# lh3/minigraph

Measured on NVIDIA H100. Metric: mapped Gbp/s (-cx lr), higher is better.
Workload: dtype int64/u8 (fp32 chain penalties, bit-exact)

## Files before the change

### minigraph_b200/csrc/mgb_engine.cu

```cuda
#include <stdio.h>
#include <stdlib.h>
#include <string.h>
#include <math.h>
#include <vector>
#include <array>
#include <memory>
#include <algorithm>
#include <string>
#include <chrono>
#include <thread>
#include <mutex>
#include <condition_variable>
#include <functional>
#include <unordered_map>
#include "mgb_hostpool.h"

#include "../../include/mgb200.h"
#include "mgb_galign.cuh"
#include "mgb_gaf.cuh"
#include "mgb_ingest.cuh"

#ifndef MGB_HOSTSIM
#include <cuda_runtime.h>
#include "mgb_index.cuh"
// ... 2377 lines not shown
		const TestTier &t;
		int32_t *smem;
		MG_HD void put(int i, int64_t rc, int64_t s, int64_t n_iter, int64_t n_cigar, int lane) const
		{
			if (lane == 0) { int64_t *o = t.out + 4 * (int64_t)i; o[0] = rc, o[1] = s, o[2] = n_iter, o[3] = n_cigar; }
		}
		MG_HD int run(int i, Arena &A, WfTbJob *tb, int lane) const
		{
			WfResult r;
			const char *ts_i = t.ts + t.t_off[i], *qs_i = t.qs + t.q_off[i];
			int64_t cont_cells = 0;
			const int rc = t.tier == 1? wfa_smem<WfTier1::W_, WfTier1::MAXLEN_, WfTier1::TBCAP_>(A, smem, t.tl[i], ts_i, t.ql[i], qs_i, &r, lane)
					: t.tier == 2? wfa_smem<WfTier2::W_, WfTier2::MAXLEN_, WfTier2::TBCAP_>(A, smem, t.tl[i], ts_i, t.ql[i], qs_i, &r, lane)
								 : wfa_smem<WfTier2::W_, WfTier2::MAXLEN_, WfTier2::TBCAP_, true>(A, smem, t.tl[i], ts_i, t.ql[i], qs_i, &r, lane, &cont_cells);
			if (rc == 1) put(i, 1, -1, 0, 0, lane);
			if (rc != 0) return rc < 0? rc : 0;
			wfa_tb_keep(tb, r, t.tl[i], ts_i, t.ql[i], qs_i, i, lane);
			return 1;
		}
		MG_HD int done(const WfTbJob &b, int lane) const
		{
			if (b.rc < 0) return b.rc;
			if (b.n_cigar > t.cap) return MGB_E_INTERNAL;
			for (int32_t j = lane; j < b.n_cigar; j += MGB_W) t.cigar[b.job * t.cap + j] = b.cig[b.first + j];
			put((int)b.job, 0, b.s, b.n_iter, b.n_cigar, lane);
			return 0;
		}
		MG_HD void fail(int i, int rc, int lane) const { put(i, rc, -1, 0, 0, lane); }
		MG_HD void traced(unsigned long long, int) const {}
	};
	MG_HD int operator()(int w, int32_t *smem, Arena &A, int, int lane) const
	{
		const Gaps g{*this, smem};
		WfaBatch<Gaps> batch;
		batch.open(A);
		for (int i = w; i < n; i += n_workers) batch.add(g, i, A, lane);
		batch.flush(g, A, lane);
		warp_sync();
		return 0;
	}
};

static int test_wfa_tier_impl(int tier, int n, const char *ts, const int64_t *t_off, const int32_t *tl, const char *qs, const int64_t *q_off,
							  const int32_t *ql, int64_t *out, uint32_t *cigar, int cap)
{
	if ((tier != 1 && tier != 2 && tier != MGB_TEST_TIER2_CONT) || n < 0 || cap < 0) {
		set_error("mgb_test_wfa_tier: tier must be 1, 2 or MGB_TEST_TIER2_CONT, n and cap at least 0");
		return MGB_E_UNSUPPORTED;
	}
	for (int i = 0; i < n; ++i)
		if (tl[i] < 1 || ql[i] < 1 || t_off[i] < 0 || q_off[i] < 0) { set_error("mgb_test_wfa_tier: gap " + std::to_string(i) + " has an empty side"); return MGB_E_UNSUPPORTED; }
	if (n == 0) return 0;
	if (int e = test_no_device()) return e;
	auto ts_d = upload(ts, test_seq_bytes(n, t_off, tl)), qs_d = upload(qs, test_seq_bytes(n, q_off, ql));
	auto t_off_d = upload(t_off, n), q_off_d = upload(q_off, n);
	auto tl_d = upload(tl, n), ql_d = upload(ql, n);
	DevBuf<int64_t> out_d(4 * (size_t)n);
	DevBuf<uint32_t> cigar_d((size_t)n * cap + 1);
	TestTier t;
	const int warps = tier == 1? StageSpec<S_WFA_SMALL>::warps : StageSpec<S_WFA_MID>::warps;
	t.tier = tier, t.cap = cap, t.n = n, t.n_workers = (std::min(n, 64 * warps) + warps - 1) / warps * warps;
	t.ts = ts_d, t.qs = qs_d, t.t_off = t_off_d, t.q_off = q_off_d, t.tl = tl_d, t.ql = ql_d, t.out = out_d, t.cigar = cigar_d;
	const uint64_t arena_bytes = tier == MGB_TEST_TIER2_CONT? (uint64_t)5 << 20 : (uint64_t)256 << 10;
	const int rc = tier == 1? test_launch<S_WFA_SMALL>(t.n_workers, t.n_workers, arena_bytes, t)
							: test_launch<S_WFA_MID>(t.n_workers, t.n_workers, arena_bytes, t);
	if (rc) return rc;
	d2h(out, out_d, sizeof(int64_t) * 4 * (size_t)n);
	d2h(cigar, cigar_d, sizeof(uint32_t) * (size_t)n * cap);
	return 0;
}

extern "C" int mgb_test_wfa_tier(int tier, int n, const char *ts, const int64_t *t_off, const int32_t *tl, const char *qs, const int64_t *q_off,
								 const int32_t *ql, int64_t *out, uint32_t *cigar, int cap)
{
	try { return test_wfa_tier_impl(tier, n, ts, t_off, tl, qs, q_off, ql, out, cigar, cap); } catch (const MgbError &e) { return e.code; }
}

struct TestGwfa {
	GraphDev g;
	int mode, walk_cap;
	const char *q;
	const int64_t *q_off;
	const int32_t *ql, *off0, *off1, *max_ed;
	const uint32_t *v0, *v1;
	int64_t *out;
	int32_t *walk;
	MG_HD int operator()(int i, int32_t *smem, Arena &A, int, int lane) const
	{
		GwfShared *sh = (GwfShared*)smem;
		GwfOpt opt;
		opt.traceback = 1, opt.max_chk = 1000, opt.bw_dyn = 1000, opt.max_lag = max_ed[i] / 2, opt.s_term = -1;
		opt.i_term = 500000000LL;
		A.top = 0, A.peak = 0;
		const char *q_i = q + q_off[i];
		int rc = 0;
		GwfResult rs;
		const GwfResult *r = &rs;
		if (mode == 0) {
			if (lane == 0) sh->A = A;
			warp_sync();
			rc = gwf_align_w(sh, g, opt, ql[i], q_i, v0[i], off0[i], v1[i], off1[i], max_ed[i], lane);
			r = &sh->r;
		} else {
			if (lane == 0) rc = gwf_align(A, g, opt, ql[i], q_i, v0[i], off0[i], v1[i], off1[i], max_ed[i], &rs);
			rc = warp_bcast_i32(rc, 0);
		}
		if (lane == 0) {
			int64_t *o = out + 6 * (int64_t)i;
			const int32_t nv = rc == 0 && r->s >= 0? r->nv : 0;
			if (nv > walk_cap) rc = MGB_E_INTERNAL;
			o[0] = rc;
			o[1] = rc == 0? r->s : -1, o[2] = rc == 0? (int64_t)r->end_v : -1, o[3] = rc == 0? r->end_off : -1;
			o[4] = rc == 0? nv : 0, o[5] = rc == 0? r->n_iter : 0;
			if (rc == 0) for (int32_t j = 0; j < nv; ++j) walk[(int64_t)i * walk_cap + j] = r->v[j];
		}
		warp_sync();
		return 0;
	}
};

static int test_gwfa_impl(const mg_idx_t *gi, int mode, int n, const char *q, const int64_t *q_off, const int32_t *ql, const uint32_t *v0,
						  const int32_t *off0, const uint32_t *v1, const int32_t *off1, const int32_t *max_ed, int64_t *out, int32_t *walk, int walk_cap)
{
	if (gi == 0 || (mode != 0 && mode != 1) || n < 0 || walk_cap < 0) { set_error("mgb_test_gwfa: an index, mode 0 or 1, n and walk_cap at least 0"); return MGB_E_UNSUPPORTED; }
	const Model *M = model_of(gi);
	for (int i = 0; i < n; ++i)
		if (ql[i] < 1 || q_off[i] < 0 || (v0[i] >> 1) >= (uint32_t)M->g.n_seg || (v1[i] >> 1) >= (uint32_t)M->g.n_seg || off0[i] < 0 || off0[i] >= M->seg_len[v0[i] >> 1]
			|| off1[i] < 0 || off1[i] >= M->seg_len[v1[i] >> 1]) {
			set_error("mgb_test_gwfa: bridge " + std::to_string(i) + " has an empty query or an end outside the graph");
			return MGB_E_UNSUPPORTED;
		}
	if (n == 0) return 0;
	if (int e = test_no_device(M->device)) return e;
	auto q_d = upload(q, test_seq_bytes(n, q_off, ql));
	auto q_off_d = upload(q_off, n);
	auto ql_d = upload(ql, n), off0_d = upload(off0, n), off1_d = upload(off1, n), max_ed_d = upload(max_ed, n);
	auto v0_d = upload(v0, n), v1_d = upload(v1, n);
	DevBuf<int64_t> out_d(6 * (size_t)n);
	DevBuf<int32_t> walk_d((size_t)n * walk_cap + 1);
	TestGwfa t;
	t.g = M->g, t.mode = mode, t.walk_cap = walk_cap;
	t.q = q_d, t.q_off = q_off_d, t.ql = ql_d, t.off0 = off0_d, t.off1 = off1_d, t.max_ed = max_ed_d, t.v0 = v0_d, t.v1 = v1_d, t.out = out_d, t.walk = walk_d;
	if (int e = test_launch<S_GWFA>(n, std::min(n, 8 * StageSpec<S_GWFA>::warps), (uint64_t)64 << 20, t)) return e;
	d2h(out, out_d, sizeof(int64_t) * 6 * (size_t)n);
	d2h(walk, walk_d, sizeof(int32_t) * (size_t)n * walk_cap);
	return 0;
}

extern "C" int mgb_test_gwfa(const mg_idx_t *gi, int mode, int n, const char *q, const int64_t *q_off, const int32_t *ql, const uint32_t *v0,
							 const int32_t *off0, const uint32_t *v1, const int32_t *off1, const int32_t *max_ed, int64_t *out, int32_t *walk, int walk_cap)
{
	try { return test_gwfa_impl(gi, mode, n, q, q_off, ql, v0, off0, v1, off1, max_ed, out, walk, walk_cap); } catch (const MgbError &e) { return e.code; }
}

struct TestRadix {
	u128 *a; int64_t n; int walk, hot_bytes; int32_t *rc;
	MG_HD int operator()(int, int32_t *hot, Arena &A, int, int lane) const
	{
		Arena H;
		arena_init(H, hot, hot_bytes > 0? (uint64_t)hot_bytes : 0);
		const int r = radix_sort_128x_w(hot_bytes > 0? H : A, a, n, lane, &A, walk != 0);
		if (lane == 0) *rc = r;
		return r;
	}
};

static int test_radix128_impl(u128 *a, int64_t n, int walk, int hot_bytes)
{
	if (n < 0 || hot_bytes < 0 || hot_bytes > 200 * 1024) { set_error("mgb_test_radix128: n >= 0 and 0 <= hot_bytes <= 200 KB"); return MGB_E_UNSUPPORTED; }
	if (int e = test_no_device()) return e;
	auto a_d = upload(a, n);
	DevBuf<int32_t> rc_d(1);
	TestRadix t;
	t.a = a_d, t.n = n, t.walk = walk, t.hot_bytes = hot_bytes, t.rc = rc_d;
	if (int e = test_launch<NO_STAGE>(1, 1, (uint64_t)n * 64 + (1 << 20), t, 1, hot_bytes)) return e;
	int32_t rc = 0;
	d2h(&rc, rc_d, sizeof(rc));
	if (rc == 0) d2h(a, a_d, sizeof(u128) * (size_t)n);
	return rc;
}

extern "C" int mgb_test_radix128(mg128_t *a, int64_t n, int walk, int hot_bytes)
{
	static_assert(sizeof(mg128_t) == sizeof(u128), "mg128_t and u128 are the same record");
	try { return test_radix128_impl((u128*)a, n, walk, hot_bytes); } catch (const MgbError &e) { return e.code; }
}

struct TestLchain {
	int mode;
	uint64_t slice;
	u128 *a;
	const int64_t *off;
	const int32_t *cnt;
	const LChainOpt *opt;
	int32_t *out;
	uint64_t *u;
	MG_HD int operator()(int i, int32_t *smem, Arena &A, int worker, int lane) const
	{
		A.top = 0;
		u128 *a_i = a + off[i];
		const int64_t n = cnt[i];
		const LChainOpt &co = opt[i];
		int32_t n_u = 0, n_v = 0;
		uint64_t *u_i = 0;
		int path = -1, staged = 0;
		const int rc = chain_staged(smem, slice, A, a_i, n, lane, &staged, [&](Arena &H, u128 *aw, int32_t *n_keep) {
			const int r = mode == 2? chain_run<1>(H, A, 1, co, n, aw, &n_u, &u_i, &n_v, lane, &path) : chain_run<0>(H, A, mode == 1, co, n, aw, &n_u, &u_i, &n_v, lane, &path);
			*n_keep = n_u > 0? n_v : 0;
			return r;
		});
		if (rc == 0) for (int32_t j = lane; j < n_u; j += MGB_W) u[off[i] + j] = u_i[j];
		if (lane == 0) {
			int32_t *o = out + 6 * (int64_t)i;
			o[0] = rc, o[1] = n_u, o[2] = n_v, o[3] = staged, o[4] = path, o[5] = worker;
		}
		warp_sync();
		return 0;
	}
};

static int test_lchain_impl(int mode, int n, const u128 *a, const int64_t *off, const int32_t *cnt, const mgb_lchain_opt_t *opt, int32_t *out, uint64_t *u, u128 *a_out)
{
#define MGB_SAME_FIELD(f) static_assert(offsetof(mgb_lchain_opt_t, f) == offsetof(LChainOpt, f) && sizeof(mgb_lchain_opt_t::f) == sizeof(LChainOpt::f), "mgb_lchain_opt_t and LChainOpt differ in " #f)
	MGB_SAME_FIELD(max_dist_x); MGB_SAME_FIELD(max_dist_y); MGB_SAME_FIELD(bw); MGB_SAME_FIELD(max_skip); MGB_SAME_FIELD(max_iter); MGB_SAME_FIELD(min_cnt);
	MGB_SAME_FIELD(min_sc); MGB_SAME_FIELD(pen_gap); MGB_SAME_FIELD(pen_skip); MGB_SAME_FIELD(is_cdna); MGB_SAME_FIELD(n_seg); MGB_SAME_FIELD(max_dist_inner);
	MGB_SAME_FIELD(cap_rmq_size);
#undef MGB_SAME_FIELD
	static_assert(sizeof(mgb_lchain_opt_t) == sizeof(LChainOpt), "mgb_lchain_opt_t and LChainOpt are the same record");
	if (mode < 0 || mode > 2 || n < 0) { set_error("mgb_test_lchain: mode 0, 1 or 2 and n at least 0"); return MGB_E_UNSUPPORTED; }
	int64_t max_cnt = 0;
	for (int i = 0; i < n; ++i) {
		if (cnt[i] < 0 || off[i] < 0) { set_error("mgb_test_lchain: set " + std::to_string(i) + " has a negative offset or count"); return MGB_E_UNSUPPORTED; }
		max_cnt = std::max(max_cnt, (int64_t)cnt[i]);
	}
	if (n == 0) return 0;
	if (int e = test_no_device()) return e;
	const int64_t n_a = test_seq_bytes(n, off, cnt);
	auto a_d = upload(a, n_a);
	auto off_d = upload(off, n);
	auto cnt_d = upload(cnt, n);
	auto opt_d = upload((const LChainOpt*)opt, n);
	DevBuf<int32_t> out_d(6 * (size_t)n);
	DevBuf<uint64_t> u_d((size_t)n_a + 1);
	TestLchain t;
	t.mode = mode, t.slice = mode == 2? StageSpec<S_CHAIN_RESCUE>::smem : StageSpec<S_CHAIN>::smem;
	t.a = a_d, t.off = off_d, t.cnt = cnt_d, t.opt = opt_d, t.out = out_d, t.u = u_d;
	const uint64_t arena_bytes = (uint64_t)max_cnt * 512 + ((uint64_t)1 << 20);
	const int rc = mode == 2? test_launch<S_CHAIN_RESCUE>(n, std::min(n, 2 * StageSpec<S_CHAIN_RESCUE>::warps), arena_bytes, t)
							: test_launch<S_CHAIN>(n, std::min(n, 2 * StageSpec<S_CHAIN>::warps), arena_bytes, t);
	if (rc) return rc;
	d2h(out, out_d, sizeof(int32_t) * 6 * (size_t)n);
	d2h(u, u_d, sizeof(uint64_t) * (size_t)n_a);
	d2h(a_out, a_d, sizeof(u128) * (size_t)n_a);
	return 0;
}

extern "C" int mgb_test_lchain(int mode, int n, const mg128_t *a, const int64_t *off, const int32_t *cnt, const mgb_lchain_opt_t *opt, int32_t *out,
							   uint64_t *u, mg128_t *a_out)
{
	try { return test_lchain_impl(mode, n, (const u128*)a, off, cnt, opt, out, u, (u128*)a_out); } catch (const MgbError &e) { return e.code; }
}

struct TestSketch {
	int k, w, mode;
	const char *seq;
	const int64_t *off, *pk_off, *mz_off;
	const int32_t *len;
	const uint64_t *pk;
	int32_t *out;
	u128 *mz;
	MG_HD int operator()(int i, int32_t *smem, Arena &A, int, int lane) const
	{
		A.top = 0;
		AVec<u128> mv;
		avec_init(mv);
		const char *s = seq + off[i];
		int rc = 0, path = -1;
		if (mode == 0) rc = sketch_seq_w(A, s, len[i], w, k, (uint32_t)i, mv, lane, (u128*)smem, pk_off[i] >= 0? pk + pk_off[i] : 0, &path);
		else if (lane == 0) rc = sketch_seq(A, s, len[i], w, k, (uint32_t)i, mv);
		rc = warp_bcast_i32(rc, 0);
		const int64_t n = rc == 0? (int64_t)warp_bcast_u64((uint64_t)mv.n, 0) : 0;
		if (n <= mz_off[i + 1] - mz_off[i]) {
			if (mode == 0) for (int64_t j = lane; j < n; j += MGB_W) mz[mz_off[i] + j] = mv.a[j];
			else if (lane == 0) for (int64_t j = 0; j < n; ++j) mz[mz_off[i] + j] = mv.a[j];
		}
		if (lane == 0) out[3 * (int64_t)i] = rc, out[3 * (int64_t)i + 1] = (int32_t)n, out[3 * (int64_t)i + 2] = path;
		warp_sync();
		return 0;
	}
};

static int test_sketch_impl(int k, int w, int n, const char *seq, const int64_t *off, const int32_t *len, int mode, int32_t *out, u128 *mz, const int64_t *mz_off)
{
	static_assert(SKETCH_PATH_SMEM_PK == MGB_SKETCH_PATH_SMEM_PK && SKETCH_PATH_SMEM == MGB_SKETCH_PATH_SMEM && SKETCH_PATH_ARENA == MGB_SKETCH_PATH_ARENA
				  && SKETCH_PATH_SEQ == MGB_SKETCH_PATH_SEQ, "the sketch paths of mgb200.h are mgb_seed.cuh's");
	if (k < 1 || k > 28 || w < 1 || w > 255 || (mode != 0 && mode != 1) || n < 0) {
		set_error("mgb_test_sketch: 1 <= k <= 28, 1 <= w <= 255, mode 0 or 1 and n at least 0");
		return MGB_E_UNSUPPORTED;
	}
	int32_t max_len = 0;
	for (int i = 0; i < n; ++i) {
		if (len[i] < 1 || off[i] < 0 || mz_off[i] < 0 || mz_off[i + 1] < mz_off[i]) {
			set_error("mgb_test_sketch: sequence " + std::to_string(i) + " is empty or has a bad offset");
			return MGB_E_UNSUPPORTED;
		}
		max_len = std::max(max_len, len[i]);
// ... 360 lines not shown
```

### minigraph_b200/csrc/mgb_gwfa.cuh

```cuda
#pragma once
#include "mgb_model.cuh"

namespace mgb {

static const int32_t GWF_DIAG_SHIFT = 0x40000000;

struct GwfDiag {
	uint64_t vd;
	int32_t k, len;
	uint32_t xo;
	int32_t t;
};
struct GwfIntv { uint64_t vd0, vd1; };
struct GwfTrace { int32_t v, pre; };

struct KeyDiagVd { MG_HD uint64_t operator()(const GwfDiag &p) const { return p.vd; } };
struct KeyIntvVd0 { MG_HD uint64_t operator()(const GwfIntv &p) const { return p.vd0; } };

MG_HD inline uint64_t gwf_gen_vd(uint32_t v, int32_t d) { return (uint64_t)v << 32 | (uint64_t)(uint32_t)(GWF_DIAG_SHIFT + d); }

struct U64Tab {
	uint64_t *key;
	int32_t *val, *ep;
	int32_t bits, epoch;
	int64_t n;
};

MG_HD inline uint32_t u64tab_hash(uint64_t key)
{
	key = ~key + (key << 21);
	key = key ^ key >> 24;
	key = (key + (key << 3)) + (key << 8);
	key = key ^ key >> 14;
	key = (key + (key << 2)) + (key << 4);
	key = key ^ key >> 28;
	key = key + (key << 31);
	return (uint32_t)key;
}

MG_HD MG_NOINLINE inline int u64tab_alloc(Arena &A, U64Tab &t, int bits)
{
	MGB_ALLOC(A, t.key, uint64_t, 1LL << bits);
	MGB_ALLOC(A, t.val, int32_t, 1LL << bits);
	MGB_ALLOC(A, t.ep, int32_t, 1LL << bits);
	MGB_NO_UNROLL
	for (int64_t i = 0; i < (1LL << bits); ++i) t.ep[i] = 0;
	t.bits = bits;
	return 0;
}
MG_HD inline int u64tab_init(Arena &A, U64Tab &t, int bits) { t.epoch = 1, t.n = 0; return u64tab_alloc(A, t, bits); }
MG_HD inline void u64tab_clear(U64Tab &t) { ++t.epoch, t.n = 0; }

MG_HD MG_NOINLINE inline int u64tab_grow(Arena &A, U64Tab &t)
{
	U64Tab o = t;
	MGB_TRY(u64tab_alloc(A, t, o.bits + 1));
	t.epoch = 1;
	uint64_t nmask = (1ULL << t.bits) - 1;
	MGB_NO_UNROLL
	for (int64_t i = 0; i < (1LL << o.bits); ++i) {
		if (o.ep[i] != o.epoch) continue;
		uint64_t g = u64tab_hash(o.key[i]) & nmask;
		while (t.ep[g] == t.epoch) g = (g + 1) & nmask;
		t.key[g] = o.key[i], t.val[g] = o.val[i], t.ep[g] = t.epoch;
	}
	return 0;
}

MG_HD inline int u64tab_put(Arena &A, U64Tab &t, uint64_t key, int *absent, int64_t *slot)
{
	for (;;) {
		uint64_t mask = (1ULL << t.bits) - 1, h = u64tab_hash(key) & mask;
		while (t.ep[h] == t.epoch && t.key[h] != key) h = (h + 1) & mask;
		if (t.ep[h] == t.epoch) { *absent = 0, *slot = (int64_t)h; return 0; }
		if ((uint64_t)(t.n + 1) * 2 > (1ULL << t.bits)) {
			MGB_TRY(u64tab_grow(A, t));
			continue;
		}
		t.key[h] = key, t.val[h] = 0, t.ep[h] = t.epoch, ++t.n;
		*absent = 1, *slot = (int64_t)h;
		return 0;
	}
}

struct GwfOpt { int32_t traceback, bw_dyn, max_lag, max_chk, s_term; int64_t i_term; };

struct GwfResult {
	int32_t s;
	uint32_t end_v;
	int32_t end_off, wlen, nv;
	int64_t n_iter;
	int32_t *v;
};

struct GwfState {
	const GraphDev *g;
	int32_t ql;
	const char *q;
	AVec<GwfDiag> a, B, ooo, Q;
	int64_t q_head;
	AVec<GwfIntv> intv, tmp, swap;
	AVec<GwfTrace> t;
	U64Tab ha, ht;
	int32_t s, end_tb;
};

MG_HD inline int gwf_trace_push(Arena &A, GwfState &z, int32_t v, int32_t pre, int32_t *idx)
{
	uint64_t key = (uint64_t)(uint32_t)v << 32 | (uint32_t)pre;
	int absent; int64_t slot;
	MGB_TRY(u64tab_put(A, z.ht, key, &absent, &slot));
	if (absent) {
		GwfTrace x; x.v = v, x.pre = pre;
		MGB_TRY(avec_push_c(A, z.t, x));
		z.ht.val[slot] = (int32_t)z.t.n - 1;
	}
	*idx = z.ht.val[slot];
	return 0;
}

MG_HD inline int gwf_diag_push(Arena &A, AVec<GwfDiag> &B, uint32_t v, int32_t d, int32_t k, uint32_t x, uint32_t ooo, int32_t t)
{
	GwfDiag p;
	p.vd = gwf_gen_vd(v, d), p.k = k, p.len = 0, p.xo = x << 1 | ooo, p.t = t;
	return avec_push_c(A, B, p);
}

MG_HD inline int32_t gwf_diag_update(GwfDiag *p, uint32_t v, int32_t d, int32_t k, uint32_t x, uint32_t ooo, int32_t t)
{
	uint64_t vd = gwf_gen_vd(v, d);
	if (p->vd == vd) {
		p->xo = p->k > k? p->xo : x << 1 | ooo;
		p->t = p->k > k? p->t : t;
		p->k = p->k > k? p->k : k;
		return 0;
	}
	return 1;
}

MG_HD inline int32_t gwf_extend1(int32_t d, int32_t k, int32_t vl, const char *ts, int32_t ql, const char *qs)
{
	int32_t max_k = (ql - d < vl? ql - d : vl) - 1;
	const char *ts_ = ts + 1, *qs_ = qs + d + 1;
	while (k + 4 <= max_k) {
		uint32_t x = ld32_unaligned(ts_ + k) ^ ld32_unaligned(qs_ + k);
		if (x) return k + (ctz32(x) >> 3);
		k += 4;
	}
	while (k < max_k && ts_[k] == qs_[k]) ++k;
	return k;
}

MG_HD MG_NOINLINE inline int gwf_sort_diag_cold(Arena &A, GwfDiag *c, int64_t n) { return radix_sort_exact(A, c, n, 8, KeyDiagVd()); }
MG_HD MG_NOINLINE inline int gwf_sort_intv_cold(Arena &A, GwfIntv *a, int64_t n) { return radix_sort_exact(A, a, n, 8, KeyIntvVd0()); }
// ... 181 lines not shown
		} else if (p->k == vl) {
			GwfIntv iv;
			iv.vd0 = gwf_gen_vd(v, d), iv.vd1 = iv.vd0 + 1;
			MGB_TRY(avec_push_c(A, z.tmp, iv));
		}
	}
	z.B.n += m;
	return 0;
}

MG_HD inline int gwf_ed_extend(Arena &A, GwfState &z, const GwfOpt &opt, uint32_t v1, int32_t off1, GwfResult *r)
{
	const GraphDev &g = *z.g;
	const int32_t ql = z.ql;
	const char *q = z.q;
	int32_t i, x, n = (int32_t)z.a.n, do_dedup = 1;
	r->end_v = (uint32_t)-1;
	r->end_off = z.end_tb = -1;
	z.tmp.n = 0;
	u64tab_clear(z.ha);
	z.Q.n = 0, z.q_head = 0;
	z.B.n = 0;
	MGB_TRY(avec_reserve_c(A, z.B, (int64_t)n * 2));
	GwfDiag *a = z.a.a;
	for (x = 0, i = 1; i <= n; ++i) {
		if (i == n || a[i].vd != a[i-1].vd + 1) {
			MGB_TRY(gwf_extend_batch(A, z, i - x, &a[x]));
			x = i;
		}
	}
	if (z.Q.n == 0) do_dedup = 0;

	while (z.q_head < z.Q.n) {
		GwfDiag t = z.Q.a[z.q_head++];
		uint32_t v, x0;
		int32_t ooo, d, k, vl;
		ooo = t.xo & 1, v = (uint32_t)(t.vd >> 32);
		d = (int32_t)t.vd - GWF_DIAG_SHIFT;
		k = t.k;
		vl = g_vlen(g, v);
		k = gwf_extend1(d, k, vl, g_vseq(g, v), ql, q);
		i = k + d;
		x0 = (t.xo >> 1) + ((uint32_t)(k - t.k) << 1);

		if (k + 1 < vl && i + 1 < ql) {
			int32_t push1 = 1, push2 = 1;
			if (z.B.n >= 2) push1 = gwf_diag_update(&z.B.a[z.B.n - 2], v, d-1, k+1, x0 + 1, ooo, t.t);
			if (z.B.n >= 1) push2 = gwf_diag_update(&z.B.a[z.B.n - 1], v, d,   k+1, x0 + 2, ooo, t.t);
			if (push1)          MGB_TRY(gwf_diag_push(A, z.B, v, d-1, k+1, x0 + 1, 1, t.t));
			if (push2 || push1) MGB_TRY(gwf_diag_push(A, z.B, v, d,   k+1, x0 + 2, 1, t.t));
			MGB_TRY(gwf_diag_push(A, z.B, v, d+1, k, x0 + 1, ooo, t.t));
		} else if (i + 1 < ql) {
			int32_t nv = g_arc_n(g, v), j, n_ext = 0, tw = -1;
			const DevArc *av = g_arc_a(g, v);
			GwfIntv iv;
			iv.vd0 = gwf_gen_vd(v, d), iv.vd1 = iv.vd0 + 1;
			MGB_TRY(avec_push_c(A, z.tmp, iv));
			if (opt.traceback) MGB_TRY(gwf_trace_push(A, z, (int32_t)v, t.t, &tw));
			for (j = 0; j < nv; ++j) {
				uint32_t w = av[j].w;
				int32_t ol = av[j].ow;
				int absent; int64_t slot;
				MGB_TRY(u64tab_put(A, z.ha, (uint64_t)w << 32 | (uint64_t)(uint32_t)(i + 1), &absent, &slot));
				if (q[i + 1] == g_vseq(g, w)[ol]) {
					++n_ext;
					if (absent) {
						GwfDiag p;
						p.vd = gwf_gen_vd(w, i + 1 - ol), p.k = ol, p.xo = (x0 + 2) << 1 | 1, p.t = tw, p.len = 0;
						MGB_TRY(avec_push_c(A, z.Q, p));
					}
				} else if (absent) {
					MGB_TRY(gwf_diag_push(A, z.B, w, i - ol,     ol, x0 + 1, 1, tw));
					MGB_TRY(gwf_diag_push(A, z.B, w, i + 1 - ol, ol, x0 + 2, 1, tw));
				}
			}
			if (nv == 0 || n_ext != nv)
				MGB_TRY(gwf_diag_push(A, z.B, v, d+1, k, x0 + 1, 1, t.t));
		} else if (v1 == (uint32_t)-1 || (v == v1 && k == off1)) {
			r->end_v = v, r->end_off = k, r->wlen = (int32_t)(x0 - (uint32_t)i - 1), z.end_tb = t.t;
			z.a.n = 0;
			return 0;
		} else if (k + 1 < vl) {
			MGB_TRY(gwf_diag_push(A, z.B, v, d-1, k+1, x0 + 1, ooo, t.t));
		} else if (v != v1) {
			int32_t nv = g_arc_n(g, v), j, tw = -1;
			const DevArc *av = g_arc_a(g, v);
			if (opt.traceback) MGB_TRY(gwf_trace_push(A, z, (int32_t)v, t.t, &tw));
			for (j = 0; j < nv; ++j)
				MGB_TRY(gwf_diag_push(A, z.B, av[j].w, i - av[j].ow, av[j].ow, x0 + 1, 1, tw));
		}
	}
	n = (int32_t)z.B.n;
	if (do_dedup) MGB_TRY(gwf_dedup(A, z, n, z.B.a, &n));
	if (opt.max_lag > 0 && n > opt.max_chk && ((z.s + 1) & 0xf) == 0)
		n = gwf_prune(n, z.B.a, (uint32_t)opt.max_lag, opt.bw_dyn);
	z.B.n = n;
	{ AVec<GwfDiag> sw = z.a; z.a = z.B; z.B = sw; }
	return 0;
}

MG_HD inline int gwf_align(Arena &A, const GraphDev &g, const GwfOpt &opt, int32_t ql, const char *q, uint32_t v0, int32_t off0,
						   uint32_t v1, int32_t off1, int32_t s_term, GwfResult *r)
{
	uint64_t mark = A.top;
	GwfState z;
	z.g = &g, z.ql = ql, z.q = q, z.s = 0, z.end_tb = -1, z.q_head = 0;
	avec_init(z.a), avec_init(z.B), avec_init(z.ooo), avec_init(z.Q), avec_init(z.intv), avec_init(z.tmp), avec_init(z.swap), avec_init(z.t);
	uint64_t mark_keep = mark;
	MGB_TRY(u64tab_init(A, z.ha, 6));
	MGB_TRY(u64tab_init(A, z.ht, 6));
	MGB_TRY(avec_reserve_c(A, z.t, 16));
	{
		GwfDiag d0;
		d0.vd = gwf_gen_vd(v0, -off0), d0.k = off0 - 1, d0.xo = 0, d0.len = 0, d0.t = 0;
		if (opt.traceback) MGB_TRY(gwf_trace_push(A, z, -1, -1, &d0.t));
		MGB_TRY(avec_push_c(A, z.a, d0));
	}
	if (s_term < 0 && opt.s_term >= 0) s_term = opt.s_term;
	r->n_iter = 0, r->nv = 0, r->v = 0, r->end_v = (uint32_t)-1, r->end_off = -1, r->wlen = 0;
	while (z.a.n > 0) {
		MGB_TRY(gwf_ed_extend(A, z, opt, v1, off1, r));
		r->n_iter += z.a.n;
		if (r->end_off >= 0 || z.a.n == 0) break;
		if (s_term >= 0 && z.s >= s_term) break;
		if (opt.i_term > 0 && r->n_iter > opt.i_term) break;
		++z.s;
	}
	if (opt.traceback && r->end_off >= 0) {
		int32_t i = z.end_tb, n = 1;
		while (i >= 0 && z.t.a[i].v >= 0) ++n, i = z.t.a[i].pre;
		int32_t *tmpw, *walk = (int32_t*)(A.base + mark);
		MGB_ALLOC(A, tmpw, int32_t, n);
		i = z.end_tb, n = 0;
		tmpw[n++] = (int32_t)r->end_v;
		while (i >= 0 && z.t.a[i].v >= 0) tmpw[n++] = z.t.a[i].v, i = z.t.a[i].pre;
		r->nv = n;
		for (i = 0; i < n >> 1; ++i) { int32_t x = tmpw[i]; tmpw[i] = tmpw[n - 1 - i], tmpw[n - 1 - i] = x; }
		for (i = 0; i < n; ++i) { int32_t x = tmpw[i]; walk[i] = x; }
		r->v = walk;
		mark_keep = mark + (((uint64_t)n * 4 + 15) & ~(uint64_t)15);
	}
	r->s = r->end_v != (uint32_t)-1? z.s : -1;
	A.top = mark_keep;
	return 0;
}


struct GwfShared {
	Arena A;
	GwfState z;
	GwfResult r;
};

MG_HD inline int gwf_extend_batch_w(GwfShared *sh, int32_t n, GwfDiag *a, int lane)
{
	GwfState &z = sh->z;
	const GraphDev &g = *z.g;
	const uint32_t v = (uint32_t)(a->vd >> 32);
	const int32_t vl = g_vlen(g, v), ql = z.ql;
	const char *ts = g_vseq(g, v);
	MGB_NO_UNROLL
	for (int32_t j = lane; j < n; j += MGB_W) {
		GwfDiag p = a[j];
		int32_t k = gwf_extend1((int32_t)p.vd - GWF_DIAG_SHIFT, p.k, vl, ts, ql, z.q);
		p.len = k - p.k;
		p.xo += (uint32_t)p.len << 2;
		p.k = k;
		a[j] = p;
	}
	int rc = 0;
	if (lane == 0) {
		rc = avec_reserve_c(sh->A, z.B, z.B.n + n + 2);
		if (rc == 0) rc = avec_reserve_c(sh->A, z.Q, z.Q.n + n);
		if (rc == 0) rc = avec_reserve_c(sh->A, z.tmp, z.tmp.n + n + 2);
	}
	warp_sync();
	rc = warp_bcast_i32(rc, 0);
	if (rc < 0) return rc;
	GwfDiag *b = &z.B.a[z.B.n];
	GwfDiag *Q = z.Q.a;
	GwfIntv *T = z.tmp.a;
	int64_t qn = z.Q.n, tn = z.tmp.n;
	int32_t m = 0;
	MGB_NO_UNROLL
	for (int32_t base = 0; base < n + 2; base += MGB_W) {
		const int32_t j = base + lane;
		GwfDiag p;
		int keep = 0, ends = 0;
		p.vd = 0, p.k = 0, p.xo = 0, p.t = 0, p.len = 0;
		if (j < n + 2) {
			if (j == 0) {
				p.vd = a[0].vd - 1, p.xo = a[0].xo + 2, p.k = a[0].k + 1, p.t = a[0].t;
			} else if (j == n + 1) {
				p.vd = a[n-1].vd + 1, p.xo = a[n-1].xo + 2, p.k = a[n-1].k, p.t = a[n-1].t;
			} else if (j == 1) {
				const int first = n == 1 || a[0].k > a[1].k;
				p.vd = a[0].vd;
				p.xo = first? a[0].xo + 4 : a[1].xo + 2;
				p.t = first? a[0].t : a[1].t;
				p.k = (first? a[0].k : a[1].k) + 1;
			} else if (j == n) {
				const int first = a[n-2].k > a[n-1].k + 1;
				p.vd = a[n-1].vd;
				p.xo = first? a[n-2].xo + 2 : a[n-1].xo + 4;
				p.t = first? a[n-2].t : a[n-1].t;
				p.k = first? a[n-2].k : a[n-1].k + 1;
			} else {
				const GwfDiag l = a[j-2], c = a[j-1], rr = a[j];
				uint32_t x = l.xo + 2;
				int32_t k = l.k, t = l.t;
				x = k > c.k + 1? x : c.xo + 4;
				t = k > c.k + 1? t : c.t;
				k = k > c.k + 1? k : c.k + 1;
				x = k > rr.k + 1? x : rr.xo + 2;
				t = k > rr.k + 1? t : rr.t;
				k = k > rr.k + 1? k : rr.k + 1;
				p.vd = c.vd, p.k = k, p.xo = x, p.t = t;
			}
			const int32_t d = (int32_t)p.vd - GWF_DIAG_SHIFT;
			if (d + p.k < ql && p.k < vl) keep = 1;
			else if (p.k == vl) ends = 1;
		}
		const uint32_t mk = warp_ballot(keep), me = warp_ballot(ends);
		if (keep) b[m + mask_rank(mk, lane)] = p;
		if (ends) {
			GwfIntv iv;
			iv.vd0 = gwf_gen_vd(v, (int32_t)p.vd - GWF_DIAG_SHIFT), iv.vd1 = iv.vd0 + 1;
			T[tn + mask_rank(me, lane)] = iv;
		}
		m += mask_count(mk), tn += mask_count(me);
	}
	MGB_NO_UNROLL
	for (int32_t base = 0; base < n; base += MGB_W) {
		const int32_t j = base + lane;
		GwfDiag p;
		int f = 0;
		p.vd = 0, p.k = 0, p.xo = 0, p.t = 0, p.len = 0;
		if (j < n) {
			p = a[j];
			f = p.k == vl - 1 || (int32_t)p.vd - GWF_DIAG_SHIFT + p.k == ql - 1;
		}
		const uint32_t mq = warp_ballot(f);
		if (f) {
			p.xo |= 1;
			a[j].xo = p.xo;
			Q[qn + mask_rank(mq, lane)] = p;
		}
		qn += mask_count(mq);
	}
	warp_sync();
	if (lane == 0) z.B.n += m, z.Q.n = qn, z.tmp.n = tn;
	warp_sync();
	return 0;
}

MG_HD inline int gwf_ed_queue(Arena &A, GwfState &z, const GwfOpt &opt, uint32_t v1, int32_t off1, GwfResult *r, int *want_dedup)
{
	const GraphDev &g = *z.g;
	const int32_t ql = z.ql;
	const char *q = z.q;
	int32_t i, n, do_dedup = z.Q.n != 0;
	MGB_NO_UNROLL
	while (z.q_head < z.Q.n) {
		GwfDiag t = z.Q.a[z.q_head++];
		uint32_t v, x0;
		int32_t ooo, d, k, vl;
		ooo = t.xo & 1, v = (uint32_t)(t.vd >> 32);
		d = (int32_t)t.vd - GWF_DIAG_SHIFT;
		k = t.k;
		vl = g_vlen(g, v);
		k = gwf_extend1(d, k, vl, g_vseq(g, v), ql, q);
		i = k + d;
		x0 = (t.xo >> 1) + ((uint32_t)(k - t.k) << 1);
		if (k + 1 < vl && i + 1 < ql) {
			int32_t push1 = 1, push2 = 1;
			if (z.B.n >= 2) push1 = gwf_diag_update(&z.B.a[z.B.n - 2], v, d-1, k+1, x0 + 1, ooo, t.t);
			if (z.B.n >= 1) push2 = gwf_diag_update(&z.B.a[z.B.n - 1], v, d,   k+1, x0 + 2, ooo, t.t);
			if (push1)          MGB_TRY(gwf_diag_push(A, z.B, v, d-1, k+1, x0 + 1, 1, t.t));
			if (push2 || push1) MGB_TRY(gwf_diag_push(A, z.B, v, d,   k+1, x0 + 2, 1, t.t));
			MGB_TRY(gwf_diag_push(A, z.B, v, d+1, k, x0 + 1, ooo, t.t));
		} else if (i + 1 < ql) {
			int32_t nv = g_arc_n(g, v), j, n_ext = 0, tw = -1;
			const DevArc *av = g_arc_a(g, v);
			GwfIntv iv;
			iv.vd0 = gwf_gen_vd(v, d), iv.vd1 = iv.vd0 + 1;
			MGB_TRY(avec_push_c(A, z.tmp, iv));
			if (opt.traceback) MGB_TRY(gwf_trace_push(A, z, (int32_t)v, t.t, &tw));
			MGB_NO_UNROLL
			for (j = 0; j < nv; ++j) {
				uint32_t w = av[j].w;
				int32_t ol = av[j].ow;
				int absent; int64_t slot;
				MGB_TRY(u64tab_put(A, z.ha, (uint64_t)w << 32 | (uint64_t)(uint32_t)(i + 1), &absent, &slot));
				if (q[i + 1] == g_vseq(g, w)[ol]) {
					++n_ext;
					if (absent) {
						GwfDiag p;
						p.vd = gwf_gen_vd(w, i + 1 - ol), p.k = ol, p.xo = (x0 + 2) << 1 | 1, p.t = tw, p.len = 0;
						MGB_TRY(avec_push_c(A, z.Q, p));
					}
				} else if (absent) {
					MGB_TRY(gwf_diag_push(A, z.B, w, i - ol,     ol, x0 + 1, 1, tw));
					MGB_TRY(gwf_diag_push(A, z.B, w, i + 1 - ol, ol, x0 + 2, 1, tw));
				}
			}
			if (nv == 0 || n_ext != nv)
				MGB_TRY(gwf_diag_push(A, z.B, v, d+1, k, x0 + 1, 1, t.t));
		} else if (v1 == (uint32_t)-1 || (v == v1 && k == off1)) {
			r->end_v = v, r->end_off = k, r->wlen = (int32_t)(x0 - (uint32_t)i - 1), z.end_tb = t.t;
			z.a.n = 0;
			*want_dedup = -1;
			return 0;
		} else if (k + 1 < vl) {
			MGB_TRY(gwf_diag_push(A, z.B, v, d-1, k+1, x0 + 1, ooo, t.t));
		} else if (v != v1) {
			int32_t nv = g_arc_n(g, v), j, tw = -1;
			const DevArc *av = g_arc_a(g, v);
			if (opt.traceback) MGB_TRY(gwf_trace_push(A, z, (int32_t)v, t.t, &tw));
			MGB_NO_UNROLL
			for (j = 0; j < nv; ++j)
				MGB_TRY(gwf_diag_push(A, z.B, av[j].w, i - av[j].ow, av[j].ow, x0 + 1, 1, tw));
		}
	}
	(void)n;
	*want_dedup = do_dedup;
	return 0;
}

MG_HD inline void gwf_ed_finish(GwfState &z, const GwfOpt &opt)
{
	int32_t n = (int32_t)z.B.n;
	if (opt.max_lag > 0 && n > opt.max_chk && ((z.s + 1) & 0xf) == 0)
		n = gwf_prune(n, z.B.a, (uint32_t)opt.max_lag, opt.bw_dyn);
	z.B.n = n;
	{ AVec<GwfDiag> sw = z.a; z.a = z.B; z.B = sw; }
}

MG_HD inline int64_t gwf_lower_bound_vd(const GwfDiag *a, int64_t n, uint64_t key)
{
	int64_t lo = 0, hi = n;
	MGB_NO_UNROLL
	while (lo < hi) { int64_t mid = (lo + hi) >> 1; if (a[mid].vd < key) lo = mid + 1; else hi = mid; }
	return lo;
}
MG_HD inline int64_t gwf_upper_bound_vd(const GwfDiag *a, int64_t n, uint64_t key)
{
	int64_t lo = 0, hi = n;
	MGB_NO_UNROLL
	while (lo < hi) { int64_t mid = (lo + hi) >> 1; if (a[mid].vd <= key) lo = mid + 1; else hi = mid; }
	return lo;
}

MG_HD inline int gwf_dedup_w(GwfShared *sh, int lane)
{
	GwfState &z = sh->z;
	Arena &A = sh->A;
	const int64_t n_old = z.intv.n, n_new = z.tmp.n;
	int rc0 = 0, tmp_big_unsorted = 0;
	if (n_new > 1) {
		GwfIntv *tn = z.tmp.a;
		int uns = 0;
		MGB_NO_UNROLL
		for (int64_t i = 1 + lane; i < n_new; i += MGB_W) if (tn[i-1].vd0 > tn[i].vd0) uns = 1;
		uns = warp_any(uns);
		if (uns && n_new <= 64) small_sort_stable_w(tn, n_new, KeyIntvVd0(), lane);
		else tmp_big_unsorted = uns;
	}
	if (lane == 0) {
		int rc = 0;
		if (n_new > 0) {
			if (tmp_big_unsorted) rc = gwf_sort_intv_cold(A, z.tmp.a, n_new);
			if (rc == 0) rc = avec_reserve_c(A, z.swap, n_old);
			if (rc == 0) z.swap.n = n_old, rc = avec_reserve_c(A, z.intv, n_old + n_new);
		}
		if (rc == 0) rc = avec_reserve_c(A, z.ooo, z.B.n);
		rc0 = rc;
	}
	warp_sync();
	rc0 = warp_bcast_i32(rc0, 0);
	if (rc0 < 0) return rc0;
	if (n_new > 0) {
		GwfIntv *b = z.swap.a, *c = z.tmp.a, *o = z.intv.a;
		MGB_NO_UNROLL
		for (int64_t i = lane; i < n_old; i += MGB_W) b[i] = o[i];
		warp_sync();
		MGB_NO_UNROLL
		for (int64_t x = lane; x < n_old; x += MGB_W) {
			const uint64_t key = b[x].vd0;
			int64_t lo = 0, hi = n_new;
			MGB_NO_UNROLL
			while (lo < hi) { int64_t mid = (lo + hi) >> 1; if (c[mid].vd0 < key) lo = mid + 1; else hi = mid; }
			o[x + lo] = b[x];
		}
		MGB_NO_UNROLL
		for (int64_t y = lane; y < n_new; y += MGB_W) {
			const uint64_t key = c[y].vd0;
			int64_t lo = 0, hi = n_old;
			MGB_NO_UNROLL
			while (lo < hi) { int64_t mid = (lo + hi) >> 1; if (b[mid].vd0 <= key) lo = mid + 1; else hi = mid; }
			o[y + lo] = c[y];
		}
		warp_sync();
		const int64_t n_m = n_old + n_new;
		int64_t k = 0;
		uint64_t carry = 0;
		MGB_NO_UNROLL
		for (int64_t base = 0; base < n_m; base += MGB_W) {
			const int64_t i = base + lane;
			GwfIntv e;
			e.vd0 = e.vd1 = 0;
			if (i < n_m) e = o[i];
			uint64_t pm = warp_incl_scan_max_u64(i < n_m? e.vd1 : 0, lane);
			if (pm < carry) pm = carry;
			uint64_t before = warp_shfl_up1_u64(pm);
			if (lane == 0) before = carry;
			const int head = i < n_m && (i == 0 || e.vd0 > before);
			const uint32_t mh = warp_ballot(head);
			if (head) {
				const int64_t g = k + mask_rank(mh, lane);
				o[g].vd0 = e.vd0;
				if (g > 0) o[g - 1].vd1 = before;
			}
			k += mask_count(mh);
			carry = warp_bcast_u64(pm, MGB_W - 1);
			warp_sync();
		}
		if (lane == 0) o[k - 1].vd1 = carry, z.intv.n = k;
		warp_sync();
	}
	GwfDiag *a = z.B.a;
	const int32_t n_a = (int32_t)z.B.n;
	int unsorted = 0;
	MGB_NO_UNROLL
	for (int32_t i = 1 + lane; i < n_a; i += MGB_W) if (a[i-1].vd > a[i].vd) unsorted = 1;
	unsorted = warp_any(unsorted);
	if (unsorted) {
		GwfDiag *b = z.ooo.a;
		int32_t n_c = 0;
		MGB_NO_UNROLL
		for (int32_t base = 0; base < n_a; base += MGB_W) {
			const int32_t i = base + lane;
			n_c += mask_count(warp_ballot(i < n_a && (a[i].xo & 1)));
		}
		const int32_t n_b = n_a - n_c;
		GwfDiag *c = b + n_b;
		int32_t jb = 0, jc = 0;
		MGB_NO_UNROLL
		for (int32_t base = 0; base < n_a; base += MGB_W) {
			const int32_t i = base + lane;
			GwfDiag p;
			p.vd = 0, p.k = 0, p.xo = 0, p.t = 0, p.len = 0;
			if (i < n_a) p = a[i];
			const uint32_t mc = warp_ballot(i < n_a && (p.xo & 1)), mb = warp_ballot(i < n_a && !(p.xo & 1));
			if (i < n_a) {
				if (p.xo & 1) c[jc + mask_rank(mc, lane)] = p;
				else b[jb + mask_rank(mb, lane)] = p;
			}
			jc += mask_count(mc), jb += mask_count(mb);
		}
		warp_sync();
		if (n_c <= 64) small_sort_stable_w(c, n_c, KeyDiagVd(), lane);
		else {
			if (lane == 0) rc0 = gwf_sort_diag_cold(A, c, n_c);
			warp_sync();
			rc0 = warp_bcast_i32(rc0, 0);
			if (rc0 < 0) return rc0;
		}
		MGB_NO_UNROLL
		for (int32_t j = lane; j < n_c; j += MGB_W) c[j].xo &= 0xfffffffeU;
		warp_sync();
		MGB_NO_UNROLL
		for (int32_t i = lane; i < n_b; i += MGB_W) a[i + gwf_lower_bound_vd(c, n_c, b[i].vd)] = b[i];
		MGB_NO_UNROLL
		for (int32_t j = lane; j < n_c; j += MGB_W) a[j + gwf_upper_bound_vd(b, n_b, c[j].vd)] = c[j];
		warp_sync();
	}
	int32_t n = 0;
	MGB_NO_UNROLL
	for (int32_t base = 0; base < n_a; base += MGB_W) {
		const int32_t i = base + lane;
		GwfDiag best;
		int head = 0;
		best.vd = 0, best.k = 0, best.xo = 0, best.t = 0, best.len = 0;
		if (i < n_a) {
			best = a[i];
			head = i == 0 || a[i-1].vd != best.vd;
			if (head)
				MGB_NO_UNROLL
				for (int32_t j = i + 1; j < n_a && a[j].vd == best.vd; ++j)
					if (best.k < a[j].k) best = a[j];
		}
		const uint32_t mh = warp_ballot(head);
		warp_sync();
		if (head) a[n + mask_rank(mh, lane)] = best;
		n += mask_count(mh);
		warp_sync();
	}
	if (z.intv.n > 0) {
		const GwfIntv *iv = z.intv.a;
		const int64_t n_iv = z.intv.n;
		int32_t k = 0;
		MGB_NO_UNROLL
		for (int32_t base = 0; base < n; base += MGB_W) {
			const int32_t i = base + lane;
			GwfDiag p;
			int keep = 0;
			p.vd = 0, p.k = 0, p.xo = 0, p.t = 0, p.len = 0;
			if (i < n) {
				p = a[i];
				int64_t lo = 0, hi = n_iv;
				MGB_NO_UNROLL
				while (lo < hi) { int64_t mid = (lo + hi) >> 1; if (iv[mid].vd0 <= p.vd) lo = mid + 1; else hi = mid; }
				keep = !(lo > 0 && p.vd < iv[lo - 1].vd1);
			}
			const uint32_t mk = warp_ballot(keep);
			warp_sync();
			if (keep) a[k + mask_rank(mk, lane)] = p;
			k += mask_count(mk);
			warp_sync();
		}
		n = k;
	}
	warp_sync();
	if (lane == 0) z.B.n = n;
	warp_sync();
	return 0;
}

MG_HD inline int gwf_align_w(GwfShared *sh, const GraphDev &g, const GwfOpt &opt, int32_t ql, const char *q, uint32_t v0, int32_t off0,
							 uint32_t v1, int32_t off1, int32_t s_term, int lane)
{
	Arena &A = sh->A;
	GwfState &z = sh->z;
	GwfResult *r = &sh->r;
	const uint64_t mark = A.top;
	if (s_term < 0 && opt.s_term >= 0) s_term = opt.s_term;
	int code = 0, go = 0;
	if (lane == 0) {
		int rc = 0;
		z.g = &g, z.ql = ql, z.q = q, z.s = 0, z.end_tb = -1, z.q_head = 0;
		avec_init(z.a), avec_init(z.B), avec_init(z.ooo), avec_init(z.Q), avec_init(z.intv), avec_init(z.tmp), avec_init(z.swap), avec_init(z.t);
		rc = u64tab_init(A, z.ha, 6);
		if (rc == 0) rc = u64tab_init(A, z.ht, 6);
		if (rc == 0) rc = avec_reserve_c(A, z.t, 16);
		if (rc == 0 && A.cap >= (1u << 16)) {
			rc = avec_reserve_c(A, z.a, 96);
			if (rc == 0) rc = avec_reserve_c(A, z.B, 192);
			if (rc == 0) rc = avec_reserve_c(A, z.ooo, 192);
			if (rc == 0) rc = avec_reserve_c(A, z.Q, 96);
			if (rc == 0) rc = avec_reserve_c(A, z.tmp, 64);
			if (rc == 0) rc = avec_reserve_c(A, z.intv, 64);
			if (rc == 0) rc = avec_reserve_c(A, z.swap, 64);
			if (rc == 0) rc = avec_reserve_c(A, z.t, 64);
		}
		if (rc == 0) {
			GwfDiag d0;
			d0.vd = gwf_gen_vd(v0, -off0), d0.k = off0 - 1, d0.xo = 0, d0.len = 0, d0.t = 0;
			if (opt.traceback) rc = gwf_trace_push(A, z, -1, -1, &d0.t);
			if (rc == 0) rc = avec_push_c(A, z.a, d0);
		}
		r->n_iter = 0, r->nv = 0, r->v = 0, r->end_v = (uint32_t)-1, r->end_off = -1, r->wlen = 0;
		code = rc, go = rc == 0 && z.a.n > 0;
	}
	warp_sync();
	code = warp_bcast_i32(code, 0), go = warp_bcast_i32(go, 0);
	MGB_NO_UNROLL
	while (go) {
		if (lane == 0) {
			r->end_v = (uint32_t)-1;
			r->end_off = z.end_tb = -1;
			z.tmp.n = 0;
			u64tab_clear(z.ha);
			z.Q.n = 0, z.q_head = 0;
			z.B.n = 0;
			code = avec_reserve_c(A, z.B, z.a.n * 2);
		}
		warp_sync();
		code = warp_bcast_i32(code, 0);
		if (code < 0) break;
		{
			const int32_t n = (int32_t)z.a.n;
			GwfDiag *a = z.a.a;
			int32_t x = 0, rc = 0;
			MGB_NO_UNROLL
			for (int32_t base = 1; base <= n && rc == 0; base += MGB_W) {
				const int32_t i = base + lane;
				uint32_t mask = warp_ballot(i <= n && (i == n || a[i].vd != a[i-1].vd + 1));
				MGB_NO_UNROLL
				while (mask && rc == 0) {
					const int32_t e = base + ctz32(mask);
					mask &= mask - 1;
					rc = gwf_extend_batch_w(sh, e - x, &a[x], lane);
					x = e;
				}
			}
			if (rc < 0) { code = rc; break; }
		}
		int dd = 0;
		if (lane == 0) code = gwf_ed_queue(A, z, opt, v1, off1, r, &dd);
		warp_sync();
		code = warp_bcast_i32(code, 0), dd = warp_bcast_i32(dd, 0);
		if (code < 0) break;
		if (dd > 0 && (code = gwf_dedup_w(sh, lane)) < 0) break;
		if (lane == 0) {
			if (dd >= 0) gwf_ed_finish(z, opt);
			go = 1;
			r->n_iter += z.a.n;
			if (r->end_off >= 0 || z.a.n == 0) go = 0;
			else if (s_term >= 0 && z.s >= s_term) go = 0;
			else if (opt.i_term > 0 && r->n_iter > opt.i_term) go = 0;
			else ++z.s;
		}
		warp_sync();
		go = warp_bcast_i32(go, 0);
	}
	warp_sync();
	if (code < 0) { if (lane == 0) A.top = mark; warp_sync(); return code; }
	if (lane == 0) {
		uint64_t mark_keep = mark;
		int rc = 0;
		if (opt.traceback && r->end_off >= 0) {
			int32_t i = z.end_tb, n = 1;
			MGB_NO_UNROLL
			while (i >= 0 && z.t.a[i].v >= 0) ++n, i = z.t.a[i].pre;
			int32_t *walk = (int32_t*)(A.base + mark);
			int32_t *tmpw = (int32_t*)arena_alloc(A, (uint64_t)n * sizeof(int32_t));
			if (tmpw == 0) rc = MGB_E_ARENA;
			else {
				i = z.end_tb, n = 0;
				tmpw[n++] = (int32_t)r->end_v;
				MGB_NO_UNROLL
				while (i >= 0 && z.t.a[i].v >= 0) tmpw[n++] = z.t.a[i].v, i = z.t.a[i].pre;
				r->nv = n;
				MGB_NO_UNROLL
				for (i = 0; i < n >> 1; ++i) { int32_t t = tmpw[i]; tmpw[i] = tmpw[n - 1 - i], tmpw[n - 1 - i] = t; }
				MGB_NO_UNROLL
				for (i = 0; i < n; ++i) { int32_t t = tmpw[i]; walk[i] = t; }
				r->v = walk;
				mark_keep = mark + (((uint64_t)n * 4 + 15) & ~(uint64_t)15);
			}
		}
		r->s = r->end_v != (uint32_t)-1? z.s : -1;
		A.top = rc == 0? mark_keep : mark;
		code = rc;
	}
	warp_sync();
	return warp_bcast_i32(code, 0);
}

}
```

Measured before the change: 1.548.

## Extend all GWFA diagonal runs in one warp pass instead of per-run batches

Replaces the per-run loop, which called the extend-and-expand routine once for each contiguous diagonal run, with a single warp-wide pass over the whole wavefront. Each lane detects whether its diagonal is a run head or tail and emits up to three successors. A packed inclusive warp scan computes output positions for kept diagonals, ending intervals and queue entries. This removes many small, poorly occupied warp iterations when runs are short, at the cost of more per-lane branching and a scan whose packed fields are limited to 1023 per warp step. A host-sim-only shape logger is also added for profiling.

```diff
diff --git a/minigraph_b200/csrc/mgb_engine.cu b/minigraph_b200/csrc/mgb_engine.cu
--- a/minigraph_b200/csrc/mgb_engine.cu
+++ b/minigraph_b200/csrc/mgb_engine.cu
@@ -2553,6 +2553,16 @@
 {
 	try { return test_gwfa_impl(gi, mode, n, q, q_off, ql, v0, off0, v1, off1, max_ed, out, walk, walk_cap); } catch (const MgbError &e) { return e.code; }
 }
+
+#ifdef MGB_HOSTSIM
+extern "C" int64_t mgb_sim_gwfa_shapes(int32_t *out, int64_t cap)
+{
+	const int64_t n = std::min(cap, (int64_t)gwf_shape_log.size());
+	if (n > 0) memcpy(out, gwf_shape_log.data(), sizeof(GwfShapeStep) * (size_t)n);
+	gwf_shape_log.clear();
+	return n;
+}
+#endif
 
 struct TestRadix {
 	u128 *a; int64_t n; int walk, hot_bytes; int32_t *rc;
diff --git a/minigraph_b200/csrc/mgb_gwfa.cuh b/minigraph_b200/csrc/mgb_gwfa.cuh
--- a/minigraph_b200/csrc/mgb_gwfa.cuh
+++ b/minigraph_b200/csrc/mgb_gwfa.cuh
@@ -1,5 +1,8 @@
 #pragma once
 #include "mgb_model.cuh"
+#if defined(MGB_HOSTSIM)
+#include <vector>
+#endif
 
 namespace mgb {
 
@@ -487,104 +490,103 @@
 	GwfResult r;
 };
 
-MG_HD inline int gwf_extend_batch_w(GwfShared *sh, int32_t n, GwfDiag *a, int lane)
+MG_HD inline int gwf_extend_all_w(GwfShared *sh, int32_t n, GwfDiag *a, int lane)
 {
 	GwfState &z = sh->z;
 	const GraphDev &g = *z.g;
-	const uint32_t v = (uint32_t)(a->vd >> 32);
-	const int32_t vl = g_vlen(g, v), ql = z.ql;
-	const char *ts = g_vseq(g, v);
-	MGB_NO_UNROLL
-	for (int32_t j = lane; j < n; j += MGB_W) {
-		GwfDiag p = a[j];
-		int32_t k = gwf_extend1((int32_t)p.vd - GWF_DIAG_SHIFT, p.k, vl, ts, ql, z.q);
-		p.len = k - p.k;
-		p.xo += (uint32_t)p.len << 2;
-		p.k = k;
-		a[j] = p;
+	const int32_t ql = z.ql;
+	int32_t n_run = 0;
+	MGB_NO_UNROLL
+	for (int32_t base = 0; base < n; base += MGB_W) {
+		const int32_t i = base + lane;
+		int head = 0;
+		if (i < n) {
+			const uint64_t vd = a[i].vd;
+			const uint32_t v = (uint32_t)(vd >> 32);
+			const int32_t k0 = a[i].k, k = gwf_extend1((int32_t)vd - GWF_DIAG_SHIFT, k0, g_vlen(g, v), g_vseq(g, v), ql, z.q);
+			a[i].len = k - k0, a[i].xo += (uint32_t)(k - k0) << 2, a[i].k = k;
+			head = i == 0 || vd != a[i-1].vd + 1;
+		}
+		n_run += mask_count(warp_ballot(head));
 	}
 	int rc = 0;
 	if (lane == 0) {
-		rc = avec_reserve_c(sh->A, z.B, z.B.n + n + 2);
+		rc = avec_reserve_c(sh->A, z.B, z.B.n + n + 2 * n_run);
 		if (rc == 0) rc = avec_reserve_c(sh->A, z.Q, z.Q.n + n);
-		if (rc == 0) rc = avec_reserve_c(sh->A, z.tmp, z.tmp.n + n + 2);
+		if (rc == 0) rc = avec_reserve_c(sh->A, z.tmp, z.tmp.n + n + 2 * n_run);
 	}
 	warp_sync();
 	rc = warp_bcast_i32(rc, 0);
 	if (rc < 0) return rc;
-	GwfDiag *b = &z.B.a[z.B.n];
-	GwfDiag *Q = z.Q.a;
-	GwfIntv *T = z.tmp.a;
-	int64_t qn = z.Q.n, tn = z.tmp.n;
-	int32_t m = 0;
-	MGB_NO_UNROLL
-	for (int32_t base = 0; base < n + 2; base += MGB_W) {
-		const int32_t j = base + lane;
+	GwfDiag *b = &z.B.a[z.B.n], *Q = &z.Q.a[z.Q.n];
+	GwfIntv *T = &z.tmp.a[z.tmp.n];
+	int32_t m = 0, qn = 0, tn = 0;
+	MGB_NO_UNROLL
+	for (int32_t base = 0; base < n; base += MGB_W) {
+		const int32_t i = base + lane;
 		GwfDiag p;
-		int keep = 0, ends = 0;
 		p.vd = 0, p.k = 0, p.xo = 0, p.t = 0, p.len = 0;
-		if (j < n + 2) {
-			if (j == 0) {
-				p.vd = a[0].vd - 1, p.xo = a[0].xo + 2, p.k = a[0].k + 1, p.t = a[0].t;
-			} else if (j == n + 1) {
-				p.vd = a[n-1].vd + 1, p.xo = a[n-1].xo + 2, p.k = a[n-1].k, p.t = a[n-1].t;
-			} else if (j == 1) {
-				const int first = n == 1 || a[0].k > a[1].k;
-				p.vd = a[0].vd;
-				p.xo = first? a[0].xo + 4 : a[1].xo + 2;
-				p.t = first? a[0].t : a[1].t;
-				p.k = (first? a[0].k : a[1].k) + 1;
-			} else if (j == n) {
-				const int first = a[n-2].k > a[n-1].k + 1;
-				p.vd = a[n-1].vd;
-				p.xo = first? a[n-2].xo + 2 : a[n-1].xo + 4;
-				p.t = first? a[n-2].t : a[n-1].t;
-				p.k = first? a[n-2].k : a[n-1].k + 1;
+		int32_t k0 = 0, k1 = 0, k2 = 0, t0 = 0, t1 = 0, t2 = 0;
+		uint32_t x0 = 0, x1 = 0, x2 = 0;
+		int keep = 0, ends = 0, f = 0;
+		if (i < n) {
+			p = a[i];
+			const int32_t vl = g_vlen(g, (uint32_t)(p.vd >> 32)), d = (int32_t)p.vd - GWF_DIAG_SHIFT;
+			const int head = i == 0 || p.vd != a[i-1].vd + 1, tail = i == n - 1 || a[i+1].vd != p.vd + 1;
+			if (head) {
+				x0 = p.xo + 2, k0 = p.k + 1, t0 = p.t;
+				const GwfDiag r = tail? p : a[i+1];
+				const int first = tail || p.k > r.k;
+				x1 = first? p.xo + 4 : r.xo + 2, t1 = first? p.t : r.t, k1 = (first? p.k : r.k) + 1;
+			} else if (tail) {
+				const GwfDiag l = a[i-1];
+				const int first = l.k > p.k + 1;
+				x1 = first? l.xo + 2 : p.xo + 4, t1 = first? l.t : p.t, k1 = first? l.k : p.k + 1;
 			} else {
-				const GwfDiag l = a[j-2], c = a[j-1], rr = a[j];
+				const GwfDiag l = a[i-1], r = a[i+1];
 				uint32_t x = l.xo + 2;
 				int32_t k = l.k, t = l.t;
-				x = k > c.k + 1? x : c.xo + 4;
-				t = k > c.k + 1? t : c.t;
-				k = k > c.k + 1? k : c.k + 1;
-				x = k > rr.k + 1? x : rr.xo + 2;
-				t = k > rr.k + 1? t : rr.t;
-				k = k > rr.k + 1? k : rr.k + 1;
-				p.vd = c.vd, p.k = k, p.xo = x, p.t = t;
+				x = k > p.k + 1? x : p.xo + 4;
+				t = k > p.k + 1? t : p.t;
+				k = k > p.k + 1? k : p.k + 1;
+				x = k > r.k + 1? x : r.xo + 2;
+				t = k > r.k + 1? t : r.t;
+				k = k > r.k + 1? k : r.k + 1;
+				x1 = x, t1 = t, k1 = k;
 			}
-			const int32_t d = (int32_t)p.vd - GWF_DIAG_SHIFT;
-			if (d + p.k < ql && p.k < vl) keep = 1;
-			else if (p.k == vl) ends = 1;
-		}
-		const uint32_t mk = warp_ballot(keep), me = warp_ballot(ends);
-		if (keep) b[m + mask_rank(mk, lane)] = p;
-		if (ends) {
-			GwfIntv iv;
-			iv.vd0 = gwf_gen_vd(v, (int32_t)p.vd - GWF_DIAG_SHIFT), iv.vd1 = iv.vd0 + 1;
-			T[tn + mask_rank(me, lane)] = iv;
-		}
-		m += mask_count(mk), tn += mask_count(me);
-	}
-	MGB_NO_UNROLL
-	for (int32_t base = 0; base < n; base += MGB_W) {
-		const int32_t j = base + lane;
-		GwfDiag p;
-		int f = 0;
-		p.vd = 0, p.k = 0, p.xo = 0, p.t = 0, p.len = 0;
-		if (j < n) {
-			p = a[j];
-			f = p.k == vl - 1 || (int32_t)p.vd - GWF_DIAG_SHIFT + p.k == ql - 1;
-		}
-		const uint32_t mq = warp_ballot(f);
+			if (tail) x2 = p.xo + 2, k2 = p.k, t2 = p.t;
+			if (head && d - 1 + k0 < ql && k0 < vl) keep |= 1;
+			else if (head && k0 == vl) ends |= 1;
+			if (d + k1 < ql && k1 < vl) keep |= 2;
+			else if (k1 == vl) ends |= 2;
+			if (tail && d + 1 + k2 < ql && k2 < vl) keep |= 4;
+			else if (tail && k2 == vl) ends |= 4;
+			f = p.k == vl - 1 || d + p.k == ql - 1;
+		}
+		const int32_t cnt = ((keep & 1) + (keep >> 1 & 1) + (keep >> 2)) | ((ends & 1) + (ends >> 1 & 1) + (ends >> 2)) << 10 | f << 20;
+		const int32_t incl = warp_incl_scan_i32(cnt, lane), tot = warp_bcast_i32(incl, MGB_W - 1), excl = incl - cnt;
+		int32_t pk = m + (excl & 1023), pe = tn + (excl >> 10 & 1023);
+		MGB_NO_UNROLL
+		for (int c = 0; c < 3; ++c) {
+			if (!((keep | ends) >> c & 1)) continue;
+			GwfDiag e;
+			e.vd = p.vd + (uint64_t)(int64_t)(c - 1), e.len = 0;
+			e.k = c == 0? k0 : c == 1? k1 : k2, e.xo = c == 0? x0 : c == 1? x1 : x2, e.t = c == 0? t0 : c == 1? t1 : t2;
+			if (keep >> c & 1) b[pk++] = e;
+			else {
+				GwfIntv iv;
+				iv.vd0 = gwf_gen_vd((uint32_t)(p.vd >> 32), (int32_t)e.vd - GWF_DIAG_SHIFT), iv.vd1 = iv.vd0 + 1;
+				T[pe++] = iv;
+			}
+		}
 		if (f) {
 			p.xo |= 1;
-			a[j].xo = p.xo;
-			Q[qn + mask_rank(mq, lane)] = p;
-		}
-		qn += mask_count(mq);
+			Q[qn + (excl >> 20)] = p;
+		}
+		m += tot & 1023, tn += tot >> 10 & 1023, qn += tot >> 20;
 	}
 	warp_sync();
-	if (lane == 0) z.B.n += m, z.Q.n = qn, z.tmp.n = tn;
+	if (lane == 0) z.B.n += m, z.Q.n += qn, z.tmp.n += tn;
 	warp_sync();
 	return 0;
 }
@@ -862,6 +864,27 @@
 	return 0;
 }
 
+#if defined(MGB_HOSTSIM)
+struct GwfShapeStep { int32_t w, runs, queue, intv, dedup, sort_n; };
+inline std::vector<GwfShapeStep> gwf_shape_log;
+inline GwfShapeStep gwf_shape_begin(const GwfState &z)
+{
+	GwfShapeStep st = {(int32_t)z.a.n, 0, 0, 0, 0, -1};
+	for (int64_t i = 0; i < z.a.n; ++i) st.runs += i == 0 || z.a.a[i].vd != z.a.a[i-1].vd + 1;
+	return st;
+}
+inline void gwf_shape_end(const GwfState &z, GwfShapeStep st, int dd)
+{
+	st.queue = (int32_t)z.Q.n, st.intv = (int32_t)z.tmp.n, st.dedup = dd > 0;
+	if (dd > 0) {
+		int unsorted = 0, n_c = 0;
+		for (int64_t i = 0; i < z.B.n; ++i) n_c += z.B.a[i].xo & 1, unsorted |= i > 0 && z.B.a[i-1].vd > z.B.a[i].vd;
+		if (unsorted) st.sort_n = n_c;
+	}
+	gwf_shape_log.push_back(st);
+}
+#endif
+
 MG_HD inline int gwf_align_w(GwfShared *sh, const GraphDev &g, const GwfOpt &opt, int32_t ql, const char *q, uint32_t v0, int32_t off0,
 							 uint32_t v1, int32_t off1, int32_t s_term, int lane)
 {
@@ -913,29 +936,18 @@
 		warp_sync();
 		code = warp_bcast_i32(code, 0);
 		if (code < 0) break;
-		{
-			const int32_t n = (int32_t)z.a.n;
-			GwfDiag *a = z.a.a;
-			int32_t x = 0, rc = 0;
-			MGB_NO_UNROLL
-			for (int32_t base = 1; base <= n && rc == 0; base += MGB_W) {
-				const int32_t i = base + lane;
-				uint32_t mask = warp_ballot(i <= n && (i == n || a[i].vd != a[i-1].vd + 1));
-				MGB_NO_UNROLL
-				while (mask && rc == 0) {
-					const int32_t e = base + ctz32(mask);
-					mask &= mask - 1;
-					rc = gwf_extend_batch_w(sh, e - x, &a[x], lane);
-					x = e;
-				}
-			}
-			if (rc < 0) { code = rc; break; }
-		}
+#if defined(MGB_HOSTSIM)
+		const GwfShapeStep shape = gwf_shape_begin(z);
+#endif
+		if ((code = gwf_extend_all_w(sh, (int32_t)z.a.n, z.a.a, lane)) < 0) break;
 		int dd = 0;
 		if (lane == 0) code = gwf_ed_queue(A, z, opt, v1, off1, r, &dd);
 		warp_sync();
 		code = warp_bcast_i32(code, 0), dd = warp_bcast_i32(dd, 0);
 		if (code < 0) break;
+#if defined(MGB_HOSTSIM)
+		if (lane == 0) gwf_shape_end(z, shape, dd);
+#endif
 		if (dd > 0 && (code = gwf_dedup_w(sh, lane)) < 0) break;
 		if (lane == 0) {
 			if (dd >= 0) gwf_ed_finish(z, opt);
```

Measured after the change: 1.564 (median of 6 runs). 1.01x the previous value.
